# perdoch/hesaff

Measured on AMD Instinct MI355X. Metric: keypoints/sec (descriptors written), 4K grayscale batch, higher is better.
Workload: dtype f32

## Files before the change

hesaff_amd/csrc/kernels_patch.h:

```cpp
#pragma once
#include <type_traits>
#include "kernels_keypoint.h"

#define HS_PATCH_ARR 1684
#define HS_PATCH_PIX_IT 7
#define HS_NEED 82

struct PatchIO {
   DPlane image;
   float *patches;
   uint32_t h_base;
   float *trows;
   const uint32_t *row_prefix;
   uint32_t trows_cap;
   uint32_t *overflow;
};

__device__ __forceinline__ float hs_tap_inside(const HsPlaneBuf &im, float wx, float wy)
{
   const uint32_t off = ((uint32_t)(int)wy * im.pitch + (uint32_t)(int)wx) * 4u;
   wx = __builtin_amdgcn_fractf(wx);
   wy = __builtin_amdgcn_fractf(wy);
   const hs_v2u r0 = __builtin_amdgcn_raw_buffer_load_b64(im.rsrc, (int)off, 0, 0);
   const hs_v2u r1 = __builtin_amdgcn_raw_buffer_load_b64(im.rsrc, (int)off, (int)im.pitch_bytes, 0);
// ... 387 lines not shown
__device__ __forceinline__ void hs_resample_chunked(const float *__restrict__ T, int P, float scale, hs_row_taps taps, int r,
                                                    float *__restrict__ s_chunk, int chunk_rows, float *s_patch)
{
   const int tid = threadIdx.x;
   const float c0 = (float)(P >> 1);
   auto y0_of = [&](int jj) {
      const float wy = c0 + (float)(jj - (HS_PATCH >> 1)) * scale;
      return min(max((int)floorf(wy), 0), P - 2);
   };
   for (int jj0 = 0; jj0 < HS_PATCH;) {
      const int ylo = y0_of(jj0) - r;
      int jj1 = jj0;
      while (jj1 + 1 < HS_PATCH && y0_of(jj1 + 1) + r + 2 - ylo <= chunk_rows) jj1++;
      const int nrows = y0_of(jj1) + r + 2 - ylo;
      {
         const v2f *src = reinterpret_cast<const v2f *>(T + ylo * HS_NEED);
         v2f *dst = reinterpret_cast<v2f *>(s_chunk);
         const int n2 = nrows * (HS_NEED / 2);
#pragma unroll 4
         for (int i = tid; i < n2; i += 256) dst[i] = src[i];
      }
      __syncthreads();
      for (int idx = jj0 * HS_PATCH + tid; idx < (jj1 + 1) * HS_PATCH; idx += 256) {
         const int jj = hs_div_small(idx, 1.0f / (float)HS_PATCH), ii = idx - jj * HS_PATCH;
         const int j = jj - (HS_PATCH >> 1), i = ii - (HS_PATCH >> 1);
         const float rx = c0 + (float)j * 0.0f, ry = c0 + (float)j * scale;
         float wx = rx + (float)i * scale, wy = ry + (float)i * 0.0f;
         const float fx = floorf(wx), fy = floorf(wy);
         wx -= fx; wy -= fy;
         const int y0 = min(max((int)fy, 0), P - 2);
         const float *tc = s_chunk + (y0 - ylo) * HS_NEED + 2 * ii;
         auto ld = [&](int dy) { return *reinterpret_cast<const v2f *>(tc + dy * HS_NEED); };
         const v2f q0 = ld(0), q1 = ld(1);
         const float kc = taps[r];
         v2f da = kc * q0, db = kc * q1;
         v2f pj = q1, mj = q0;
#pragma unroll 4
         for (int jt = 1; jt <= r; jt++) {
            const v2f pn = ld(jt + 1), mn = ld(-jt);
            const float kj = taps[r + jt];
            const v2f sa = pj + mn, sb = pn + mj;
            da += kj * sa;
            db += kj * sb;
            pj = pn;
            mj = mn;
         }
         s_patch[idx] = (1.0f - wy) * ((1.0f - wx) * da.x + wx * da.y) + (wy) * ((1.0f - wx) * db.x + wx * db.y);
      }
      __syncthreads();
      jj0 = jj1 + 1;
   }
}

template <int NR, int NB>
__device__ __forceinline__ void hs_gather_slots(const HsPlaneBuf &img, const v2f *rc, const v2f *__restrict__ ctab, float a11, float a21, int half,
                                                int xb, int P, int r, float *__restrict__ srow, int sstride)
{
   const int lane = threadIdx.x & 63, pm = P - 1;
   float v[NR][NB];
#pragma unroll
   for (int it = 0; it < NB; it++) {
      const int xx = min(xb + lane + 64 * it, pm);
      const v2f c = ctab ? ctab[xx] : hs_col_coord(a11, a21, xx - half);
#pragma unroll
      for (int i = 0; i < NR; i++) {
         const v2f w = rc[i] + c;
         v[i][it] = hs_tap_inside(img, w.x, w.y);
      }
   }
#pragma unroll
   for (int it = 0; it < NB; it++)
#pragma unroll
      for (int i = 0; i < NR; i++) HS_KEEP(v[i][it]);
#pragma unroll
   for (int it = 0; it < NB; it++) {
      const int xx = xb + lane + 64 * it;
      if (xx < P) {
#pragma unroll
         for (int i = 0; i < NR; i++) srow[i * sstride + r + xx] = v[i][it];
      }
   }
}

template <int NR, int NIT>
__device__ __forceinline__ void hs_gather_rows(const HsPlaneBuf &img, const v2f *rc, const v2f *__restrict__ ctab, float a11, float a21, int half,
                                               int P, int r, float *__restrict__ srow, int sstride)
{
   static_assert(NIT == 1 || NIT == 2 || NIT == 4 || NIT == 8, "power of two");
   int xb = 0;
   for (; ((P - xb + 63) >> 6) >= NIT; xb += 64 * NIT)
      hs_gather_slots<NR, NIT>(img, rc, ctab, a11, a21, half, xb, P, r, srow, sstride);
   const int rem = (P - xb + 63) >> 6;
   if (NIT > 4 && (rem & 4)) { hs_gather_slots<NR, 4>(img, rc, ctab, a11, a21, half, xb, P, r, srow, sstride); xb += 256; }
   if (NIT > 2 && (rem & 2)) { hs_gather_slots<NR, 2>(img, rc, ctab, a11, a21, half, xb, P, r, srow, sstride); xb += 128; }
   if (NIT > 1 && (rem & 1)) { hs_gather_slots<NR, 1>(img, rc, ctab, a11, a21, half, xb, P, r, srow, sstride); }
}

template <int NIT>
__device__ __forceinline__ void hs_row_stream(const HsPlaneBuf &img, float x, float y, float a11, float a12, float a21, float a22, int P, int yy,
                                              float scale, const v2f *__restrict__ ctab, hs_row_taps taps, int K,
                                              float *__restrict__ srow, float *__restrict__ out82, int pad_r = 0)
{
   const int lane = threadIdx.x & 63, half = P >> 1, pm = P - 1, r = K >> 1;
   const v2f rc = hs_row_coord(x, y, a12, a22, yy - half);
   hs_gather_rows<1, NIT>(img, &rc, ctab, a11, a21, half, P, r, srow, 0);
   HS_WAVE_LDS_SYNC();
   {
      const float first = srow[r], last = srow[r + pm];
      for (int i = lane; i < r; i += 64) { srow[i] = first; srow[r + P + i] = last; }
   }
   HS_WAVE_LDS_SYNC();
   if (lane < HS_PATCH) {
      const float c0 = (float)half;
      const float w = c0 + (float)(lane - 20) * scale;
      const int x0 = min(max((int)floorf(w), 0), pm - 1);
      const float *s = srow + x0;
      auto G = [&](int jt) { v2f g; g.x = s[jt]; g.y = s[jt + 1]; return g; };
      v2f t = taps[0] * G(0);
#pragma unroll 8
      for (int jt = 1; jt < K; jt++) t += taps[jt] * G(jt);
      v2f *o = reinterpret_cast<v2f *>(out82) + lane;
      *o = t;
      if (pad_r > 0 && (yy == 0 || yy == pm)) {
         const int step = (yy == 0) ? -(HS_NEED / 2) : (HS_NEED / 2);
         for (int jr = 1; jr <= pad_r; jr++) o[jr * step] = t;
      }
   }
   HS_WAVE_LDS_SYNC();
}

template <int NIT>
__device__ __forceinline__ void hs_row_stream2(const HsPlaneBuf &img, float x, float y, float a12, float a22, int P, int yyA, int yyB,
                                               float scale, const v2f *__restrict__ ctab, hs_row_taps taps, int K,
                                               float *__restrict__ srowA, float *__restrict__ srowB, float *__restrict__ outA, float *__restrict__ outB, int pad_r,
                                               float a11 = 0.0f, float a21 = 0.0f)
{
   const int lane = threadIdx.x & 63, half = P >> 1, pm = P - 1, r = K >> 1;
   const v2f rc[2] = {hs_row_coord(x, y, a12, a22, yyA - half), hs_row_coord(x, y, a12, a22, yyB - half)};
   hs_gather_rows<2, NIT>(img, rc, ctab, a11, a21, half, P, r, srowA, (int)(srowB - srowA));
   HS_WAVE_LDS_SYNC();
   {
      const float fA = srowA[r], lA = srowA[r + pm], fB = srowB[r], lB = srowB[r + pm];
      for (int i = lane; i < r; i += 64) { srowA[i] = fA; srowA[r + P + i] = lA; srowB[i] = fB; srowB[r + P + i] = lB; }
   }
   HS_WAVE_LDS_SYNC();
   if (lane < HS_PATCH) {
      const float c0 = (float)half;
      const float w = c0 + (float)(lane - 20) * scale;
      const int x0 = min(max((int)floorf(w), 0), pm - 1);
      const float *sA = srowA + x0, *sB = srowB + x0;
      auto GA = [&](int jt) { v2f g; g.x = sA[jt]; g.y = sA[jt + 1]; return g; };
      auto GB = [&](int jt) { v2f g; g.x = sB[jt]; g.y = sB[jt + 1]; return g; };
      v2f tA = taps[0] * GA(0), tB = taps[0] * GB(0);
#pragma unroll 4
      for (int jt = 1; jt < K; jt++) {
         const float k = taps[jt];
         tA += k * GA(jt);
         tB += k * GB(jt);
      }
      v2f *oA = reinterpret_cast<v2f *>(outA) + lane, *oB = reinterpret_cast<v2f *>(outB) + lane;
      *oA = tA;
      *oB = tB;
      if (pad_r > 0 && yyA == 0)
         for (int jr = 1; jr <= pad_r; jr++) oA[-jr * (HS_NEED / 2)] = tA;
      if (pad_r > 0 && yyB == pm)
         for (int jr = 1; jr <= pad_r; jr++) oB[jr * (HS_NEED / 2)] = tB;
   }
   HS_WAVE_LDS_SYNC();
}

template <int NIT>
__device__ __forceinline__ void hs_row_stream3(const HsPlaneBuf &img, float x, float y, float a12, float a22, int P, int yy0, int yy1, int yy2,
                                               float scale, const v2f *__restrict__ ctab, hs_row_taps taps, int K,
                                               float *__restrict__ srow, int sstride, float *__restrict__ out0, float *__restrict__ out1,
                                               float *__restrict__ out2, int pad_r, float a11 = 0.0f, float a21 = 0.0f)
{
   const int lane = threadIdx.x & 63, half = P >> 1, pm = P - 1, r = K >> 1;
   const v2f rc[3] = {hs_row_coord(x, y, a12, a22, yy0 - half), hs_row_coord(x, y, a12, a22, yy1 - half),
                      hs_row_coord(x, y, a12, a22, yy2 - half)};
   float *srow1 = srow + sstride, *srow2 = srow + 2 * sstride;
   hs_gather_rows<3, NIT>(img, rc, ctab, a11, a21, half, P, r, srow, sstride);
   HS_WAVE_LDS_SYNC();
   {
      const float f0 = srow[r], l0 = srow[r + pm], f1 = srow1[r], l1 = srow1[r + pm], f2 = srow2[r], l2 = srow2[r + pm];
      for (int i = lane; i < r; i += 64) {
         srow[i] = f0; srow[r + P + i] = l0;
         srow1[i] = f1; srow1[r + P + i] = l1;
         srow2[i] = f2; srow2[r + P + i] = l2;
      }
   }
   HS_WAVE_LDS_SYNC();
   {
      const int tA = lane, tB = min(64 + lane, 3 * HS_PATCH - 1);
      const int rowA = tA >= HS_PATCH ? 1 : 0, rowB = tB >= 2 * HS_PATCH ? 2 : 1;
      const int colA = tA - HS_PATCH * rowA, colB = tB - HS_PATCH * rowB;
      const float c0 = (float)half;
      const float wA = c0 + (float)(colA - 20) * scale, wB = c0 + (float)(colB - 20) * scale;
      const int xA = min(max((int)floorf(wA), 0), pm - 1), xB = min(max((int)floorf(wB), 0), pm - 1);
      const float *sA = srow + rowA * sstride + xA, *sB = srow + rowB * sstride + xB;
      v2f tA2, tB2;
      float a0 = sA[0], a1 = sA[1], b0 = sB[0], b1 = sB[1];
      const float k0 = taps[0];
      float tA0 = k0 * a0, tA1 = k0 * a1, tB0 = k0 * b0, tB1 = k0 * b1;
#pragma unroll 4
      for (int jt = 1; jt < K; jt++) {
         const float k = taps[jt];
         a0 = a1; b0 = b1;
         a1 = sA[jt + 1]; b1 = sB[jt + 1];
         tA0 += k * a0; tA1 += k * a1;
         tB0 += k * b0; tB1 += k * b1;
      }
      tA2.x = tA0; tA2.y = tA1; tB2.x = tB0; tB2.y = tB1;
      const int yA = rowA ? yy1 : yy0, yB = rowB == 2 ? yy2 : yy1;
      v2f *oA = reinterpret_cast<v2f *>(rowA ? out1 : out0) + colA;
      v2f *oB = reinterpret_cast<v2f *>(rowB == 2 ? out2 : out1) + colB;
      *oA = tA2;
      if (64 + lane < 3 * HS_PATCH) *oB = tB2;
      if (pad_r > 0) {
         if (yA == 0) for (int jr = 1; jr <= pad_r; jr++) oA[-jr * (HS_NEED / 2)] = tA2;
         if (yA == pm) for (int jr = 1; jr <= pad_r; jr++) oA[jr * (HS_NEED / 2)] = tA2;
         if (64 + lane < 3 * HS_PATCH) {
            if (yB == 0) for (int jr = 1; jr <= pad_r; jr++) oB[-jr * (HS_NEED / 2)] = tB2;
            if (yB == pm) for (int jr = 1; jr <= pad_r; jr++) oB[jr * (HS_NEED / 2)] = tB2;
         }
      }
   }
   HS_WAVE_LDS_SYNC();
}

#define HS_MID_PMAX 128
#define HS_MID_SROW 160
#define HS_BIG_SROW 640
#define HS_BIG_TAPS 128
#define HS_MID_RPAD 14
#define HS_BIG_RPAD 57
#define HS_CHUNK_MIN_ROWS 4
#define HS_MID_NIT3_BIG 2
#define HS_MID_NIT3_SMALL 1
#define HS_MID_BLOCKS (256 * 7)
#define HS_BIG_BLOCKS (256 * 8)

template <int PMAX> struct MidGeom {
   static constexpr bool BIG = PMAX > HS_MID_PMAX;
   static constexpr int SROW = BIG ? HS_BIG_SROW : HS_MID_SROW;
   static constexpr int NTAP = BIG ? HS_BIG_TAPS : 32;
   static constexpr int RPAD = BIG ? HS_BIG_RPAD : HS_MID_RPAD;
   static constexpr int CHUNK_MIN = BIG ? 0 : 64;
   static constexpr int SROWS = 12 * SROW > CHUNK_MIN * HS_NEED ? 12 * SROW : CHUNK_MIN * HS_NEED;
   static constexpr int CHUNK_ROWS = SROWS / HS_NEED;
   static constexpr int FLOATS = HS_PATCH_ARR + NTAP + 2 * (PMAX + 2) + SROWS;
};

template <int PMAX>
__global__ __launch_bounds__(256) void k_patch_mid(HessList hl, PatchWork pw, PatchIO io, KpTables tb)
{
   typedef MidGeom<PMAX> GM;
   constexpr int BIN = GM::BIG ? 3 : 2;
   constexpr int NIT = GM::BIG ? 4 : 2;
   constexpr int NIT3 = GM::BIG ? HS_MID_NIT3_BIG : HS_MID_NIT3_SMALL;
   extern __shared__ __attribute__((aligned(16))) float smem[];
   float *s_patch = smem;
   v2f *s_C = reinterpret_cast<v2f *>(s_patch + HS_PATCH_ARR + GM::NTAP);
   float *s_srow = reinterpret_cast<float *>(s_C + (PMAX + 2));
   float *Tp = io.trows + (size_t)blockIdx.x * ((size_t)(PMAX + 2 * GM::RPAD) * HS_NEED);

   const int tid = threadIdx.x, wave = tid >> 6;
   const uint32_t cnt = min(pw.bin_count[BIN], pw.cap);
   const int imPitch = io.image.pitch;

   __shared__ uint32_t s_item;
   for (;;) {
      if (tid == 0) s_item = atomicAdd(pw.bin_work + BIN, 1u);
      __syncthreads();
      const uint32_t wi = (uint32_t)__builtin_amdgcn_readfirstlane((int)s_item);
      if (wi >= cnt) break;
      const uint32_t h = pw.bin_items[(size_t)BIN * pw.cap + wi];
      const int b = hl.meta[h] >> 8;
      const HsPlaneBuf ib = hs_plane_buf(io.image.img(b), io.image.rows, imPitch);
      const float x = hl.x[h], y = hl.y[h];
      const float a11 = pw.A[4 * h], a12 = pw.A[4 * h + 1], a21 = pw.A[4 * h + 2], a22 = pw.A[4 * h + 3];
      const int P0 = pw.P0[h], P = P0 + 2, half = P >> 1;
      const float scale = (float)P0 / (float)HS_PATCH;
      const int K = tb.patch_tap_k[(P0 - 1) >> 1];
      const float *taps_g = tb.patch_taps + tb.patch_tap_off[(P0 - 1) >> 1];
      const hs_row_taps ktap = HS_ROW_TAPS(taps_g);
      for (int m = tid; m < P; m += 256) s_C[m] = hs_col_coord(a11, a21, m - half);
      __syncthreads();
      float *srowA = s_srow + wave * 3 * GM::SROW, *srowB = srowA + GM::SROW;
#pragma unroll 1
      for (int yy = wave; yy < P; yy += 12) {
         const int rr = K >> 1;
         if (yy + 8 < P)
            hs_row_stream3<NIT3>(ib, x, y, a12, a22, P, yy, yy + 4, yy + 8, scale, s_C, ktap, K, srowA, GM::SROW,
                                 Tp + (size_t)(yy + rr) * HS_NEED, Tp + (size_t)(yy + 4 + rr) * HS_NEED, Tp + (size_t)(yy + 8 + rr) * HS_NEED, rr);
         else if (yy + 4 < P)
            hs_row_stream2<NIT>(ib, x, y, a12, a22, P, yy, yy + 4, scale, s_C, ktap, K, srowA, srowB,
                                Tp + (size_t)(yy + (K >> 1)) * HS_NEED, Tp + (size_t)(yy + 4 + (K >> 1)) * HS_NEED, K >> 1);
         else
            hs_row_stream<NIT>(ib, x, y, a11, a12, a21, a22, P, yy, scale, s_C, ktap, K, srowA,
                               Tp + (size_t)(yy + (K >> 1)) * HS_NEED, K >> 1);
      }
      __syncthreads();
      if ((float)(K + 1) + (float)(HS_CHUNK_MIN_ROWS - 1) * scale <= (float)GM::CHUNK_ROWS)
         hs_resample_chunked(Tp + (K >> 1) * HS_NEED, P, scale, ktap, K >> 1, s_srow, GM::CHUNK_ROWS, s_patch);
      else
         hs_resample_reduced_batched<true>(Tp + (K >> 1) * HS_NEED, P, scale, ktap, K >> 1, s_patch);
      __syncthreads();
      for (int i = tid; i < HS_PATCH_PIX; i += 256) {
         float *po = io.patches + (size_t)(h - io.h_base) * HS_PATCH_PIX + i;
         hs_store_nt(po, s_patch[i]);
      }
      __syncthreads();
   }
}

#define HS_LARGE_CHUNK 18
#define HS_LARGE_NIT3 2

__global__ __launch_bounds__(256) void k_patch_large_rows(HessList hl, PatchWork pw, PatchIO io, KpTables tb, int srow_stride, int tap_stride, int nrow,
                                                          int p_lo, int p_hi)
{
   extern __shared__ __attribute__((aligned(16))) float smem[];
   const int wave = __builtin_amdgcn_readfirstlane((int)(threadIdx.x >> 6));
   float *srow = smem + (size_t)wave * (nrow * srow_stride + tap_stride);
   const uint32_t *pre = io.row_prefix;
   const uint32_t n_items = min(pw.bin_count[HS_NBINS - 1], pw.cap);
   if (n_items == 0) return;
   const uint32_t row_hi = pre[n_items];
   if (row_hi > io.trows_cap) {
      if (threadIdx.x == 0 && blockIdx.x == 0) *io.overflow = 1u;
      return;
   }
   const int imPitch = io.image.pitch;
   const uint32_t ntasks = (row_hi + HS_LARGE_CHUNK - 1) / HS_LARGE_CHUNK;
   const uint32_t nw = blockDim.x >> 6;
   for (uint32_t task = blockIdx.x * nw + wave; task < ntasks; task += gridDim.x * nw) {
      uint32_t row = task * HS_LARGE_CHUNK;
      const uint32_t row_end = min(row + HS_LARGE_CHUNK, row_hi);
      uint32_t lo = 0, hi = n_items;
      while (hi - lo > 1) {
         const uint32_t mid = (lo + hi) >> 1;
         if (pre[mid] <= row) lo = mid; else hi = mid;
      }
      uint32_t it = lo;
      while (row < row_end) {
         const uint32_t it_rows_end = min(pre[it + 1], row_end);
         const uint32_t h = pw.bin_items[(size_t)(HS_NBINS - 1) * pw.cap + it];
         const int P0 = pw.P0[h], P = P0 + 2;
         if (P <= p_lo || P > p_hi) { row = it_rows_end; it++; continue; }
         const int b = hl.meta[h] >> 8;
         const float scale = (float)P0 / (float)HS_PATCH;
         const int K = tb.patch_tap_k[(P0 - 1) >> 1];
         const float *taps = tb.patch_taps + tb.patch_tap_off[(P0 - 1) >> 1];
         const HsPlaneBuf ib = hs_plane_buf(io.image.img(b), io.image.rows, imPitch);
         const float kx = hl.x[h], ky = hl.y[h];
         const float a11 = pw.A[4 * h], a12 = pw.A[4 * h + 1], a21 = pw.A[4 * h + 2], a22 = pw.A[4 * h + 3];
         const uint32_t first = pre[it];
         const hs_row_taps ktap = HS_ROW_TAPS(taps);
         float *const out0 = io.trows + (size_t)row * HS_NEED;
// ... 105 lines not shown
```

hesaff_amd/csrc/pipeline.hip:

```cpp
#include <hip/hip_runtime.h>
#include <algorithm>
#include <atomic>
#include <chrono>
#include <cmath>
#include <cstdio>
#include <cstdlib>
#include <cstring>
#include <string>
#include <vector>
#include <condition_variable>
#include <deque>
#include <future>
#include <map>
#include <memory>
#include <mutex>
#include <thread>

#include "../../include/hesaff_amd.h"
#include "host_tables.h"
#include "kernels_keypoint.h"
#include "kernels_patch.h"
#include "kernels_sift.h"
#include "kernels_pyramid.h"
#include "kernels_export.h"
// ... 275 lines not shown
         if (bytes == 0 || bytes > kLargest) return nullptr;
         std::vector<std::pair<void *, size_t>> evicted;
         bool room = false;
         {
            std::lock_guard<std::mutex> lk(mu);
            for (size_t k = 0; k < parked.size(); k++)
               if (parked[k].second == bytes) { void *q = parked[k].first; parked[k] = parked.back(); parked.pop_back(); return q; }
            while (bytes_total + bytes > max_bytes && !parked.empty()) {
               evicted.push_back(parked.back());
               bytes_total -= parked.back().second;
               parked.pop_back();
            }
            room = bytes_total + bytes <= max_bytes;
            if (room) bytes_total += bytes;
         }
         for (auto &b : evicted) (void)hipHostFree(b.first);
         if (!room) return nullptr;
         void *q = nullptr;
         if (hipSetDevice(device) != hipSuccess || hipHostMalloc(&q, bytes, hipHostMallocDefault) != hipSuccess) {
            (void)hipGetLastError();
            std::lock_guard<std::mutex> lk(mu);
            bytes_total -= bytes;
            return nullptr;
         }
         return q;
      }
      void give(void *q, size_t bytes)
      {
         std::lock_guard<std::mutex> lk(mu);
         parked.emplace_back(q, bytes);
      }
      void trim(size_t keep)
      {
         std::vector<std::pair<void *, size_t>> out;
         {
            std::lock_guard<std::mutex> lk(mu);
            size_t held = 0;
            for (auto &b : parked) held += b.second;
            while (held > keep && !parked.empty()) {
               out.push_back(parked.back());
               held -= parked.back().second; bytes_total -= parked.back().second;
               parked.pop_back();
            }
         }
         for (auto &b : out) (void)hipHostFree(b.first);
      }
      ~PinReadCache() { trim(0); }
   } pin_read;
   std::vector<PinBuf> pin_out;
   hesaff_engine::BlockRing ring;
   hipStream_t h2d_stream = nullptr, d2h_stream = nullptr;
   float export_ms = 0.0f; int32_t export_rows = 0;
   PinBuf h_small_end, h_small_mid, h_small_exp;
   DevBuf t_mask_idx, t_sgrad_nb, t_sgrad_om, t_vo_rows, t_vo_src, b_rowprefix, b_trows, b_trows2, b_trows3;
   DevBuf b_jplane;
   DevBuf b_ex_len, b_ex_sums, b_ex_off, b_ex_imgoff, b_ex_starts;
   size_t rows_lds_set = 0;
   int n_cu = 256;
   uint32_t g_small0 = 256 * 6, g_small1 = 256 * 4, g_mid = HS_MID_BLOCKS, g_big = HS_BIG_BLOCKS, g_lfin = 256 * 4, g_shist = 256 * 32;
   uint32_t sgrad_grid = 256 * 32;
   uint32_t trows_rows = 4u << 20;

   hesaff_timings tm;
   int profiling = 0;
   int out_format = HESAFF_OUT_TEXT;
   int resume = 0;
   int pool_priority = -1;
   int stage_threads = 4;
   hipStream_t side_streams[HS_NSIDE] = {nullptr, nullptr, nullptr, nullptr};
   hipStream_t sift_stream = nullptr;
   hipStream_t aff_stream = nullptr;
   DevEvent ev_detect_done, ev_batch_done;
   std::vector<DevEvent> ev_aff;
   DevEvent ev_extract_done[HS_NSLOT], ev_sift_done[HS_NSLOT];
   DevBuf b_patches2[HS_NSLOT];
   DevBuf b_siftvec2, b_meanvar2, b_siftvo2;
   DevEvent ev_fork, ev_join[HS_NSIDE];
   bool fast_pyramid = false;
   bool no_overlap = false;
   bool debug = false;

   std::vector<DevEvent> ev_pool;
   size_t ev_used = 0;
};

namespace {

struct EvPair { hipEvent_t a, b; int kind; double bytes; };

hipEvent_t get_event(hesaff_ctx *c)
{
   if (c->ev_used == c->ev_pool.size()) c->ev_pool.emplace_back(hipEventDefault);
   return c->ev_pool[c->ev_used++];
}

template <class T> void upload(DevBuf &b, const std::vector<T> &v)
{
   b.ensure(std::max<size_t>(v.size() * sizeof(T), 16));
   HIP_TRY(hipMemcpy(b.p, v.data(), v.size() * sizeof(T), hipMemcpyHostToDevice));
}

void build_tables(hesaff_ctx *c)
{
   std::vector<float> smm(HS_SMM_PIX), sm(HS_PATCH_PIX), w0(HS_PATCH), w1(HS_PATCH);
   std::vector<int32_t> b0(HS_PATCH), b1(HS_PATCH);
   hesaff::gauss_mask(HS_SMM, smm.data());
   hesaff::circ_gauss_mask(HS_PATCH, sm.data());
// ... 209 lines not shown
         }
   }
   const int ppitch0 = round_up(PW, 64);
   const size_t pplane0 = (size_t)B * PH * ppitch0;
   if (c->up) {
      c->geo.b_up.ensure(pplane0 * 4);
      c->upimg = make_plane(c->geo.b_up.as<float>(), PH, PW, ppitch0);
   }
   c->geo.b_L3.ensure(pplane0 * 4);
   c->geo.b_R.ensure(pplane0 * 4 * 5);
   {
      const void *before = c->geo.b_map.p;
      const size_t before_bytes = c->geo.b_map.bytes;
      c->geo.b_map.ensure(std::max<size_t>((size_t)B * PH * PW * 4, 16));
      if (c->geo.b_map.p != before || c->geo.b_map.bytes != before_bytes) c->map_clean = false;
      int kb = 1;
      while (kb < 32 && (3ull * (unsigned long long)PH * PW) > (1ull << kb)) kb++;
      if (kb != c->map_kbits) { c->map_kbits = kb; c->map_clean = false; }
   }
   const long long total_words = (long long)B * words;
   c->geo.b_bitmask.ensure(std::max<size_t>((size_t)total_words * 8, 16));
   c->geo.b_prefix.ensure(std::max<size_t>((size_t)(total_words + 1) * 4, 16));
   double mpx = (double)B * PH * PW / 1.0e6;
   double capd = mpx * (double)c->par.max_kpts_per_mpx;
   if (capd < 4096) capd = 4096;
   if (capd > 2.0e9) throw HsError(HESAFF_ERR_ARG, "batch too large for 32-bit keypoint indices");
   c->cap = ((uint32_t)capd + 63u) & ~63u;
   const size_t cap = c->cap;
   const long long scan_items = std::max<long long>(total_words, (long long)cap);
   c->geo.b_blocksums.ensure((size_t)((scan_items + SCAN_BLOCK - 1) / SCAN_BLOCK + 1) * 4);
   c->b_counters.ensure(64 * 4);
   {
      const unsigned long long waves0 = (unsigned long long)((PW + EXM_STRIP - 1) / EXM_STRIP) * (unsigned long long)(PH / 32 + 1) * (unsigned long long)B;
      const unsigned long long cc = (unsigned long long)cap + (unsigned long long)cap / 8 + HS_CAND_BLOCK * waves0;
      if (cc > 0xfffffff0ull) throw HsError(HESAFF_ERR_ARG, "batch too large for 32-bit candidate indices");
      c->cand_cap = (uint32_t)cc;
      c->geo.b_cand.ensure((size_t)cc * sizeof(CandRec));
   }
   c->geo.b_rec_f.ensure(cap * 4 * 4);
   c->geo.b_rec_i.ensure(cap * 4 * 4);
   c->geo.b_rec_w.ensure(cap * 8);
   c->geo.b_hess_f.ensure(cap * 4 * 4);
   c->geo.b_hess_i.ensure(cap * 2 * 4);
   c->geo.b_aff.ensure(cap * 6 * 4);
   c->geo.b_pw.ensure(cap * 6 * 4);
   c->geo.b_bins.ensure(cap * HS_NBINS * 4);
   c->geo.b_rank.ensure((cap + 1) * 4);
   c->geo.b_desc.ensure(cap * 128);
   c->geo.b_out.ensure(cap * sizeof(KeyRec));
   c->geo.b_starts.ensure(((size_t)(B + 1) * 3 + 2) * 4);
   const int max_p0 = (int)std::floor(std::sqrt((double)W * (double)H)) + 3;
   ensure_patch_taps(c, max_p0);
   refresh_tables_struct(c);
   c->b_trows2.ensure((size_t)HS_MID_BLOCKS * (HS_MID_PMAX + 2 * HS_MID_RPAD) * HS_NEED * 4);
   c->b_trows3.ensure((size_t)HS_BIG_BLOCKS * (HS_BIN3_PMAX + 2 * HS_BIG_RPAD) * HS_NEED * 4);
   {
      const LargeGeom lg = large_geom(c->max_p0 + 2);
      if (lg.lds / 4 > HS_LDS_PER_CU) throw HsError(HESAFF_ERR_ARG, "image too large for the large-window row kernel (sqrt(width x height) above about 27900)");
      const size_t want = std::min<size_t>(lg.lds + (size_t)8 * lg.srow_stride * 4, HS_LDS_PER_CU);
      if (want > c->rows_lds_set) {
         set_dyn_lds(k_patch_large_rows, want);
         c->rows_lds_set = want;
      }
   }
   c->B = B; c->H = H; c->W = W;
}

template <class LOAD> void exclusive_scan(hesaff_ctx *c, LOAD load, long long n, uint32_t *out, uint32_t *total)
{
   if (n <= 0) { HIP_TRY(hipMemsetAsync(total, 0, 4, c->stream)); return; }
   const int nb = (int)((n + SCAN_BLOCK - 1) / SCAN_BLOCK);
   uint32_t *bs = c->geo.b_blocksums.as<uint32_t>();
   hipLaunchKernelGGL(k_scan_reduce<LOAD>, dim3(nb), dim3(256), 0, c->stream, load, n, bs);
   hipLaunchKernelGGL(k_scan_sums, dim3(1), dim3(256), 0, c->stream, bs, nb, total);
   hipLaunchKernelGGL(k_scan_down<LOAD>, dim3(nb), dim3(256), 0, c->stream, load, n, bs, out);
}

struct StageTimer {
   hesaff_ctx *c;
   std::vector<EvPair> pairs;
   std::vector<hipStream_t> streams;
   explicit StageTimer(hesaff_ctx *ctx) : c(ctx) {}
   int begin(int kind, double bytes = 0, hipStream_t st = nullptr)
   {
      if (!c->profiling) return -1;
      if (kind >= 100 && c->profiling < 2) return -1;
      if (!st) st = c->stream;
      EvPair p; p.a = get_event(c); p.b = get_event(c); p.kind = kind; p.bytes = bytes;
      (void)hipEventRecord(p.a, st);
      pairs.push_back(p);
      streams.push_back(st);
      return (int)pairs.size() - 1;
   }
   void end(int id) { if (id >= 0) (void)hipEventRecord(pairs[id].b, streams[id]); }
};

enum { T_PYR = 0, T_DET = 1, T_AFF = 2, T_PATCH = 3, T_SIFT = 4, T_TOTAL = 5, T_PACK = 6, T_BLURHESS = 100, T_EXTREMA = 101 };

template <int K, bool WL, bool WR, bool WH, bool WR0 = false, int SRC = SRC_PLANE>
void launch_march(hesaff_ctx *c, const DPlane &in, const DPlane &outL, const DPlane &outR, const DPlane &outHalf, const float *taps,
                  float norm2, int B, const DPlane &outR0 = DPlane(), float norm2_in = 0.0f, const GraySrc &gs = GraySrc(), const DPlane &outGray = DPlane())
{
   const int strips = (in.cols + BM_STRIP - 1) / BM_STRIP;
   const long long blocks_per_band = (long long)((strips + 3) / 4) * B;
   int best_nb = 16 * (int)std::max<long long>(1, std::min<long long>(4, 64 / std::max<long long>(1, blocks_per_band)));
   best_nb = std::max(1, std::min(best_nb, std::max(1, in.rows / 8)));
   const int band = (in.rows + best_nb - 1) / best_nb;
// ... 58 lines not shown
   uint32_t *cnt = c->b_counters.as<uint32_t>();
   const size_t cap = c->cap;
   s.counters = cnt;
   s.cl.count = cnt + 0; s.cl.items = c->geo.b_cand.as<CandRec>(); s.cl.cap = c->cand_cap; s.cl.overflow = cnt + 2;
   s.rl.count = cnt + 1; s.rl.cap = c->cap;
   float *rf = c->geo.b_rec_f.as<float>();
   s.rl.x = rf; s.rl.y = rf + cap; s.rl.s = rf + 2 * cap; s.rl.response = rf + 3 * cap;
   uint32_t *ri = c->geo.b_rec_i.as<uint32_t>();
   s.rl.meta = (int32_t *)ri; s.rl.cell = ri + cap; s.rl.key = ri + 2 * cap; s.rl.bit = ri + 3 * cap;
   s.rl.word = c->geo.b_rec_w.as<long long>();
   float *hf = c->geo.b_hess_f.as<float>();
   s.hl.x = hf; s.hl.y = hf + cap; s.hl.s = hf + 2 * cap; s.hl.response = hf + 3 * cap;
   int32_t *hi = c->geo.b_hess_i.as<int32_t>();
   s.hl.meta = hi; s.hl.r0c0 = hi + cap; s.hl.cap = c->cap;
   int32_t *ai = c->geo.b_aff.as<int32_t>();
   s.ao.converged = ai; s.ao.iters = ai + cap; s.ao.U = (float *)(ai + 2 * cap);
   int32_t *pi = c->geo.b_pw.as<int32_t>();
   s.pw.P0 = pi; s.pw.alive = pi + cap; s.pw.A = (float *)(pi + 2 * cap);
   s.pw.bin_count = cnt + 8; s.pw.bin_work = cnt + 24; s.pw.bin_items = c->geo.b_bins.as<uint32_t>(); s.pw.cap = c->cap;
   return s;
}

void run_patch_stage(hesaff_ctx *c, const Lists &s, const DPlane &image, float *patches_out, uint32_t h_base, uint32_t large_rows_bound,
                     const PlaneTab *pt = nullptr)
{
   hipStream_t st = c->stream;
   PatchIO io;
   memset(&io, 0, sizeof io);
   io.image = image;
   io.patches = patches_out;
   io.h_base = h_base;
   if (c->fast_pyramid && pt) {
      hipStream_t s0 = st;
      const bool forked = c->side_streams[0] && !c->no_overlap;
      if (forked) {
         HIP_TRY(hipEventRecord(c->ev_fork, st));
         HIP_TRY(hipStreamWaitEvent(c->side_streams[0], c->ev_fork, 0));
         s0 = c->side_streams[0];
      }
      hipLaunchKernelGGL(k_patch_extract_small<0>, dim3(c->g_small0), dim3(256), small_extract_lds_bytes(0), s0, s.hl, s.pw, io, c->tables);
      if (forked) HIP_TRY(hipEventRecord(c->ev_join[0], s0));
      hipLaunchKernelGGL(k_patch_pyramid, dim3((uint32_t)c->n_cu * 32u), dim3(256), 0, st, s.hl, s.pw, io, *pt, (int)c->oct.size(), c->consts.pd0, 1);
      if (forked) HIP_TRY(hipStreamWaitEvent(st, c->ev_join[0], 0));
      return;
   }
   hipStream_t s0 = st, s1 = st, s2 = st, s3 = st;
   const bool forked = c->side_streams[0] && !c->no_overlap;
   if (forked) {
      HIP_TRY(hipEventRecord(c->ev_fork, st));
      for (int i = 0; i < HS_NSIDE; i++) HIP_TRY(hipStreamWaitEvent(c->side_streams[i], c->ev_fork, 0));
      s0 = c->side_streams[0]; s1 = c->side_streams[1]; s2 = c->side_streams[2]; s3 = c->side_streams[3];
   }
   {
      PatchIO io2 = io;
      io2.trows = c->b_trows2.as<float>();
      PatchIO io3 = io;
      io3.trows = c->b_trows3.as<float>();
      hipLaunchKernelGGL(k_patch_extract_small<0>, dim3(c->g_small0), dim3(256), small_extract_lds_bytes(0), s0, s.hl, s.pw, io, c->tables);
      hipLaunchKernelGGL(k_patch_extract_small<1>, dim3(c->g_small1), dim3(256), small_extract_lds_bytes(1), s1, s.hl, s.pw, io, c->tables);
      hipLaunchKernelGGL(k_patch_mid<HS_MID_PMAX>, dim3(c->g_mid), dim3(256), mid_lds_bytes(), s2, s.hl, s.pw, io2, c->tables);
      hipLaunchKernelGGL(k_patch_mid<HS_BIN3_PMAX>, dim3(c->g_big), dim3(256), big_lds_bytes(), s3, s.hl, s.pw, io3, c->tables);
   }
   if (large_rows_bound > 0) {
      const uint32_t rows_cap = std::max(large_rows_bound, c->trows_rows);
      c->b_trows.ensure((size_t)rows_cap * HS_NEED * 4);
      c->b_rowprefix.ensure(((size_t)c->cap + 1) * 4);
      const int pmax = std::min(c->max_p0 + 2, std::max(HS_BIN3_PMAX + 1, (c->batch_max_p > 0 ? c->batch_max_p : c->max_p0 + 2)));
      io.trows = c->b_trows.as<float>();
      io.row_prefix = c->b_rowprefix.as<uint32_t>();
      io.trows_cap = rows_cap;
      io.overflow = s.counters + 6;
      hipLaunchKernelGGL(k_large_prefix, dim3(1), dim3(256), 0, st, s.pw, c->b_rowprefix.as<uint32_t>());
      auto launch_rows = [&](int p_lo, int p_hi) {
         const LargeGeom lg = large_geom(std::min(c->max_p0 + 2, (p_hi + 255) / 256 * 256));
         const size_t wave1 = lg.lds / 4;
         const size_t wave3 = wave1 + (size_t)2 * lg.srow_stride * 4;
         const int nrow = wave3 * 6 <= HS_LDS_PER_CU ? 3 : 1;
         const size_t per_wave = nrow == 3 ? wave3 : wave1;
         uint32_t nw = 4;
         while (nw > 1 && per_wave * nw > HS_LDS_PER_CU) nw >>= 1;
         if (nw == 4 && (HS_LDS_PER_CU / (per_wave * 2)) * 2 > (HS_LDS_PER_CU / (per_wave * 4)) * 4) nw = 2;
         if (nrow == 3) nw = std::min<uint32_t>(nw, HS_LARGE_NW);
         const uint32_t gblocks = std::min<uint32_t>((large_rows_bound + nw * HS_LARGE_CHUNK - 1) / (nw * HS_LARGE_CHUNK), 256 * 16 * (4 / nw));
         hipLaunchKernelGGL(k_patch_large_rows, dim3(gblocks), dim3(64 * nw), per_wave * nw, st, s.hl, s.pw, io, c->tables, lg.srow_stride, lg.tap_stride, nrow,
                            p_lo, std::min(p_hi, 0x7ffffff0));
      };
      if (pmax > HS_LARGE_SPLIT) { launch_rows(0, HS_LARGE_SPLIT); launch_rows(HS_LARGE_SPLIT, pmax); }
      else launch_rows(0, pmax);
      hipLaunchKernelGGL(k_patch_large_finish, dim3(c->g_lfin), dim3(256), 0, st, s.pw, io, c->tables);
   }
   if (forked) {
      for (int i = 0; i < HS_NSIDE; i++) HIP_TRY(hipEventRecord(c->ev_join[i], c->side_streams[i]));
      for (int i = 0; i < HS_NSIDE; i++) HIP_TRY(hipStreamWaitEvent(st, c->ev_join[i], 0));
   }
}

void run_detection(hesaff_ctx *c, const SrcImages &src, int B, const Lists &s, StageTimer &tm, bool keep_all_planes, float *planes_out,
                   bool detect = true)
{
   const hesaff::OctaveSchedule &sc = c->sched;
   hipStream_t st = c->stream;
   uint32_t *cnt = s.counters;
   const float *ptaps = c->t_pyr_taps.as<float>();
   if (detect) {
      HIP_TRY(hipMemsetAsync(cnt, 0, 64 * 4, st));
      HIP_TRY(hipMemsetAsync(c->geo.b_bitmask.p, 0, std::max<size_t>((size_t)B * c->words_per_image * 8, 8), st));
      if (!c->map_clean) { HIP_TRY(hipMemsetAsync(c->geo.b_map.p, 0xFF, c->geo.b_map.bytes, st)); c->map_epoch = c->map_kbits < 32 ? (0xffffffffu >> c->map_kbits) : 0u; c->map_clean = true; }
   }

   int t = tm.begin(T_PYR);
   DPlane none = make_plane(nullptr, 0, 0, 0);
   const bool fused_gray = !c->oct.empty() && c->pyr_K[0] == 11 && !c->up;
   if (fused_gray) {
// ... 441 lines not shown
```

Before: 38.69 million.

## Keep mid-bin transposed rows in an LDS ring and resample incrementally

For the mid-size patch kernel, the row-filtered intermediate rows are now kept in a sliding LDS window instead of a per-block global scratch buffer. Output patch rows are resampled from that window as soon as their source rows are ready, and the live rows are compacted to the front when the window fills. This removes the global write/readback round trip and the mid trows allocation. In exchange it adds extra block-wide barriers and copy passes, and it uses more LDS per block, which the code asserts still allows five blocks per CU.

Result: no change. 38.66 million (-0.1%).

```diff
diff --git a/hesaff_amd/csrc/kernels_patch.h b/hesaff_amd/csrc/kernels_patch.h
--- a/hesaff_amd/csrc/kernels_patch.h
+++ b/hesaff_amd/csrc/kernels_patch.h
@@ -463,6 +463,41 @@
    }
 }
 
+template <bool TAIL>
+__device__ __forceinline__ void hs_resample_rows_lds(const float *__restrict__ s_T, int base, int jj0, int jj1, int P, float scale, hs_row_taps taps,
+                                                     int r, float *s_patch)
+{
+   const float c0 = (float)(P >> 1);
+   for (int idx = jj0 * HS_PATCH + (int)threadIdx.x; idx < (jj1 + 1) * HS_PATCH; idx += 256) {
+      const int jj = hs_div_small(idx, 1.0f / (float)HS_PATCH), ii = idx - jj * HS_PATCH;
+      const int j = jj - (HS_PATCH >> 1), i = ii - (HS_PATCH >> 1);
+      const float rx = c0 + (float)j * 0.0f, ry = c0 + (float)j * scale;
+      float wx = rx + (float)i * scale, wy = ry + (float)i * 0.0f;
+      const float fx = floorf(wx), fy = floorf(wy);
+      wx -= fx; wy -= fy;
+      const int y0 = min(max((int)fy, 0), P - 2);
+      const float *tc = s_T + (y0 + r - base) * HS_NEED + 2 * ii;
+      const int dmax = P - 1 - y0;
+      auto ld = [&](int dy) { return *reinterpret_cast<const v2f *>(tc + dy * HS_NEED); };
+      auto ldp = [&](int dy) { return ld(TAIL ? min(dy, dmax) : dy); };
+      const v2f q0 = ld(0), q1 = ld(1);
+      const float kc = taps[r];
+      v2f da = kc * q0, db = kc * q1;
+      v2f pj = q1, mj = q0;
+#pragma unroll 4
+      for (int jt = 1; jt <= r; jt++) {
+         const v2f pn = ldp(jt + 1), mn = ld(-jt);
+         const float kj = taps[r + jt];
+         const v2f sa = pj + mn, sb = pn + mj;
+         da += kj * sa;
+         db += kj * sb;
+         pj = pn;
+         mj = mn;
+      }
+      s_patch[idx] = (1.0f - wy) * ((1.0f - wx) * da.x + wx * da.y) + (wy) * ((1.0f - wx) * db.x + wx * db.y);
+   }
+}
+
 template <int NR, int NB>
 __device__ __forceinline__ void hs_gather_slots(const HsPlaneBuf &img, const v2f *rc, const v2f *__restrict__ ctab, float a11, float a21, int half,
                                                 int xb, int P, int r, float *__restrict__ srow, int sstride)
@@ -510,7 +545,7 @@
 template <int NIT>
 __device__ __forceinline__ void hs_row_stream(const HsPlaneBuf &img, float x, float y, float a11, float a12, float a21, float a22, int P, int yy,
                                               float scale, const v2f *__restrict__ ctab, hs_row_taps taps, int K,
-                                              float *__restrict__ srow, float *__restrict__ out82, int pad_r = 0)
+                                              float *__restrict__ srow, float *__restrict__ out82, int pad_r = 0, bool pad_below = true)
 {
    const int lane = threadIdx.x & 63, half = P >> 1, pm = P - 1, r = K >> 1;
    const v2f rc = hs_row_coord(x, y, a12, a22, yy - half);
@@ -532,7 +567,7 @@
       for (int jt = 1; jt < K; jt++) t += taps[jt] * G(jt);
       v2f *o = reinterpret_cast<v2f *>(out82) + lane;
       *o = t;
-      if (pad_r > 0 && (yy == 0 || yy == pm)) {
+      if (pad_r > 0 && (yy == 0 || (pad_below && yy == pm))) {
          const int step = (yy == 0) ? -(HS_NEED / 2) : (HS_NEED / 2);
          for (int jr = 1; jr <= pad_r; jr++) o[jr * step] = t;
       }
@@ -544,7 +579,7 @@
 __device__ __forceinline__ void hs_row_stream2(const HsPlaneBuf &img, float x, float y, float a12, float a22, int P, int yyA, int yyB,
                                                float scale, const v2f *__restrict__ ctab, hs_row_taps taps, int K,
                                                float *__restrict__ srowA, float *__restrict__ srowB, float *__restrict__ outA, float *__restrict__ outB, int pad_r,
-                                               float a11 = 0.0f, float a21 = 0.0f)
+                                               float a11 = 0.0f, float a21 = 0.0f, bool pad_below = true)
 {
    const int lane = threadIdx.x & 63, half = P >> 1, pm = P - 1, r = K >> 1;
    const v2f rc[2] = {hs_row_coord(x, y, a12, a22, yyA - half), hs_row_coord(x, y, a12, a22, yyB - half)};
@@ -574,7 +609,7 @@
       *oB = tB;
       if (pad_r > 0 && yyA == 0)
          for (int jr = 1; jr <= pad_r; jr++) oA[-jr * (HS_NEED / 2)] = tA;
-      if (pad_r > 0 && yyB == pm)
+      if (pad_r > 0 && pad_below && yyB == pm)
          for (int jr = 1; jr <= pad_r; jr++) oB[jr * (HS_NEED / 2)] = tB;
    }
    HS_WAVE_LDS_SYNC();
@@ -584,7 +619,8 @@
 __device__ __forceinline__ void hs_row_stream3(const HsPlaneBuf &img, float x, float y, float a12, float a22, int P, int yy0, int yy1, int yy2,
                                                float scale, const v2f *__restrict__ ctab, hs_row_taps taps, int K,
                                                float *__restrict__ srow, int sstride, float *__restrict__ out0, float *__restrict__ out1,
-                                               float *__restrict__ out2, int pad_r, float a11 = 0.0f, float a21 = 0.0f)
+                                               float *__restrict__ out2, int pad_r, float a11 = 0.0f, float a21 = 0.0f,
+                                               bool pad_below = true)
 {
    const int lane = threadIdx.x & 63, half = P >> 1, pm = P - 1, r = K >> 1;
    const v2f rc[3] = {hs_row_coord(x, y, a12, a22, yy0 - half), hs_row_coord(x, y, a12, a22, yy1 - half),
@@ -629,10 +665,10 @@
       if (64 + lane < 3 * HS_PATCH) *oB = tB2;
       if (pad_r > 0) {
          if (yA == 0) for (int jr = 1; jr <= pad_r; jr++) oA[-jr * (HS_NEED / 2)] = tA2;
-         if (yA == pm) for (int jr = 1; jr <= pad_r; jr++) oA[jr * (HS_NEED / 2)] = tA2;
+         if (pad_below && yA == pm) for (int jr = 1; jr <= pad_r; jr++) oA[jr * (HS_NEED / 2)] = tA2;
          if (64 + lane < 3 * HS_PATCH) {
             if (yB == 0) for (int jr = 1; jr <= pad_r; jr++) oB[-jr * (HS_NEED / 2)] = tB2;
-            if (yB == pm) for (int jr = 1; jr <= pad_r; jr++) oB[jr * (HS_NEED / 2)] = tB2;
+            if (pad_below && yB == pm) for (int jr = 1; jr <= pad_r; jr++) oB[jr * (HS_NEED / 2)] = tB2;
          }
       }
    }
@@ -648,18 +684,22 @@
 #define HS_CHUNK_MIN_ROWS 4
 #define HS_MID_NIT3_BIG 2
 #define HS_MID_NIT3_SMALL 1
+#define HS_MID_TROWS 52
 #define HS_MID_BLOCKS (256 * 7)
 #define HS_BIG_BLOCKS (256 * 8)
 
 template <int PMAX> struct MidGeom {
    static constexpr bool BIG = PMAX > HS_MID_PMAX;
    static constexpr int SROW = BIG ? HS_BIG_SROW : HS_MID_SROW;
-   static constexpr int NTAP = BIG ? HS_BIG_TAPS : 32;
    static constexpr int RPAD = BIG ? HS_BIG_RPAD : HS_MID_RPAD;
-   static constexpr int CHUNK_MIN = BIG ? 0 : 64;
-   static constexpr int SROWS = 12 * SROW > CHUNK_MIN * HS_NEED ? 12 * SROW : CHUNK_MIN * HS_NEED;
+   static constexpr int SROWS = 12 * SROW;
    static constexpr int CHUNK_ROWS = SROWS / HS_NEED;
-   static constexpr int FLOATS = HS_PATCH_ARR + NTAP + 2 * (PMAX + 2) + SROWS;
+   static constexpr int NTAP = BIG ? HS_BIG_TAPS : 0;
+   static constexpr int TROWS = BIG ? 0 : HS_MID_TROWS;
+   static constexpr int COPY_IT = ((2 * RPAD + 1) * (HS_NEED / 2) + 255) / 256;
+   static constexpr int FLOATS = HS_PATCH_ARR + NTAP + 2 * (PMAX + 2) + SROWS + TROWS * HS_NEED;
+   static_assert(BIG || TROWS >= 2 * RPAD + 1 + 12, "a round's rows beside the live ones");
+   static_assert(BIG || FLOATS * 4 + 256 <= 160 * 1024 / 5, "five blocks per CU");
 };
 
 template <int PMAX>
@@ -673,8 +713,8 @@
    float *s_patch = smem;
    v2f *s_C = reinterpret_cast<v2f *>(s_patch + HS_PATCH_ARR + GM::NTAP);
    float *s_srow = reinterpret_cast<float *>(s_C + (PMAX + 2));
-   float *Tp = io.trows + (size_t)blockIdx.x * ((size_t)(PMAX + 2 * GM::RPAD) * HS_NEED);
-
+   float *Tp = nullptr;
+   if constexpr (GM::BIG) Tp = io.trows + (size_t)blockIdx.x * ((size_t)(PMAX + 2 * GM::RPAD) * HS_NEED);
    const int tid = threadIdx.x, wave = tid >> 6;
    const uint32_t cnt = min(pw.bin_count[BIN], pw.cap);
    const int imPitch = io.image.pitch;
@@ -698,24 +738,71 @@
       for (int m = tid; m < P; m += 256) s_C[m] = hs_col_coord(a11, a21, m - half);
       __syncthreads();
       float *srowA = s_srow + wave * 3 * GM::SROW, *srowB = srowA + GM::SROW;
+      if constexpr (!GM::BIG) {
+         float *s_T = s_srow + GM::SROWS;
+         const int r = K >> 1;
+         const float c0 = (float)half;
+         auto y0_of = [&](int jj) {
+            const float wy = c0 + (float)(jj - (HS_PATCH >> 1)) * scale;
+            return min(max((int)floorf(wy), 0), P - 2);
+         };
+         int base = 0;
+         int jjn = 0;
 #pragma unroll 1
-      for (int yy = wave; yy < P; yy += 12) {
-         const int rr = K >> 1;
-         if (yy + 8 < P)
-            hs_row_stream3<NIT3>(ib, x, y, a12, a22, P, yy, yy + 4, yy + 8, scale, s_C, ktap, K, srowA, GM::SROW,
-                                 Tp + (size_t)(yy + rr) * HS_NEED, Tp + (size_t)(yy + 4 + rr) * HS_NEED, Tp + (size_t)(yy + 8 + rr) * HS_NEED, rr);
-         else if (yy + 4 < P)
-            hs_row_stream2<NIT>(ib, x, y, a12, a22, P, yy, yy + 4, scale, s_C, ktap, K, srowA, srowB,
-                                Tp + (size_t)(yy + (K >> 1)) * HS_NEED, Tp + (size_t)(yy + 4 + (K >> 1)) * HS_NEED, K >> 1);
+         for (int yb = 0; yb < P; yb += 12) {
+            if (yb + r + 12 - base > GM::TROWS) {
+               const int nbase = y0_of(jjn);
+               const int n2 = (yb + r - nbase) * (HS_NEED / 2);
+               const v2f *src = reinterpret_cast<const v2f *>(s_T + (nbase - base) * HS_NEED);
+               v2f *dst = reinterpret_cast<v2f *>(s_T);
+               v2f keep[GM::COPY_IT];
+#pragma unroll
+               for (int k = 0; k < GM::COPY_IT; k++)
+                  if (tid + 256 * k < n2) keep[k] = src[tid + 256 * k];
+               __syncthreads();
+#pragma unroll
+               for (int k = 0; k < GM::COPY_IT; k++)
+                  if (tid + 256 * k < n2) dst[tid + 256 * k] = keep[k];
+               base = nbase;
+            }
+            const int yy = yb + wave;
+            float *o = s_T + (yy + r - base) * HS_NEED;
+            if (yy + 8 < P)
+               hs_row_stream3<NIT3>(ib, x, y, a12, a22, P, yy, yy + 4, yy + 8, scale, s_C, ktap, K, srowA, GM::SROW,
+                                    o, o + 4 * HS_NEED, o + 8 * HS_NEED, r, 0.0f, 0.0f, false);
+            else if (yy + 4 < P)
+               hs_row_stream2<NIT>(ib, x, y, a12, a22, P, yy, yy + 4, scale, s_C, ktap, K, srowA, srowB, o, o + 4 * HS_NEED, r, 0.0f, 0.0f, false);
+            else if (yy < P)
+               hs_row_stream<NIT>(ib, x, y, a11, a12, a21, a22, P, yy, scale, s_C, ktap, K, srowA, o, r, false);
+            __syncthreads();
+            if (yb + 12 < P) {
+               int jj1 = jjn - 1;
+               while (jj1 + 1 < HS_PATCH && y0_of(jj1 + 1) + r + 1 <= yb + 11) jj1++;
+               if (jj1 >= jjn) hs_resample_rows_lds<false>(s_T, base, jjn, jj1, P, scale, ktap, r, s_patch);
+               jjn = jj1 + 1;
+            } else
+               hs_resample_rows_lds<true>(s_T, base, jjn, HS_PATCH - 1, P, scale, ktap, r, s_patch);
+         }
+      } else {
+#pragma unroll 1
+         for (int yy = wave; yy < P; yy += 12) {
+            const int rr = K >> 1;
+            if (yy + 8 < P)
+               hs_row_stream3<NIT3>(ib, x, y, a12, a22, P, yy, yy + 4, yy + 8, scale, s_C, ktap, K, srowA, GM::SROW,
+                                    Tp + (size_t)(yy + rr) * HS_NEED, Tp + (size_t)(yy + 4 + rr) * HS_NEED, Tp + (size_t)(yy + 8 + rr) * HS_NEED, rr);
+            else if (yy + 4 < P)
+               hs_row_stream2<NIT>(ib, x, y, a12, a22, P, yy, yy + 4, scale, s_C, ktap, K, srowA, srowB,
+                                   Tp + (size_t)(yy + (K >> 1)) * HS_NEED, Tp + (size_t)(yy + 4 + (K >> 1)) * HS_NEED, K >> 1);
+            else
+               hs_row_stream<NIT>(ib, x, y, a11, a12, a21, a22, P, yy, scale, s_C, ktap, K, srowA,
+                                  Tp + (size_t)(yy + (K >> 1)) * HS_NEED, K >> 1);
+         }
+         __syncthreads();
+         if ((float)(K + 1) + (float)(HS_CHUNK_MIN_ROWS - 1) * scale <= (float)GM::CHUNK_ROWS)
+            hs_resample_chunked(Tp + (K >> 1) * HS_NEED, P, scale, ktap, K >> 1, s_srow, GM::CHUNK_ROWS, s_patch);
          else
-            hs_row_stream<NIT>(ib, x, y, a11, a12, a21, a22, P, yy, scale, s_C, ktap, K, srowA,
-                               Tp + (size_t)(yy + (K >> 1)) * HS_NEED, K >> 1);
-      }
-      __syncthreads();
-      if ((float)(K + 1) + (float)(HS_CHUNK_MIN_ROWS - 1) * scale <= (float)GM::CHUNK_ROWS)
-         hs_resample_chunked(Tp + (K >> 1) * HS_NEED, P, scale, ktap, K >> 1, s_srow, GM::CHUNK_ROWS, s_patch);
-      else
-         hs_resample_reduced_batched<true>(Tp + (K >> 1) * HS_NEED, P, scale, ktap, K >> 1, s_patch);
+            hs_resample_reduced_batched<true>(Tp + (K >> 1) * HS_NEED, P, scale, ktap, K >> 1, s_patch);
+      }
       __syncthreads();
       for (int i = tid; i < HS_PATCH_PIX; i += 256) {
          float *po = io.patches + (size_t)(h - io.h_base) * HS_PATCH_PIX + i;
diff --git a/hesaff_amd/csrc/pipeline.hip b/hesaff_amd/csrc/pipeline.hip
--- a/hesaff_amd/csrc/pipeline.hip
+++ b/hesaff_amd/csrc/pipeline.hip
@@ -351,7 +351,7 @@
    hipStream_t h2d_stream = nullptr, d2h_stream = nullptr;
    float export_ms = 0.0f; int32_t export_rows = 0;
    PinBuf h_small_end, h_small_mid, h_small_exp;
-   DevBuf t_mask_idx, t_sgrad_nb, t_sgrad_om, t_vo_rows, t_vo_src, b_rowprefix, b_trows, b_trows2, b_trows3;
+   DevBuf t_mask_idx, t_sgrad_nb, t_sgrad_om, t_vo_rows, t_vo_src, b_rowprefix, b_trows, b_trows3;
    DevBuf b_jplane;
    DevBuf b_ex_len, b_ex_sums, b_ex_off, b_ex_imgoff, b_ex_starts;
    size_t rows_lds_set = 0;
@@ -667,7 +667,6 @@
    const int max_p0 = (int)std::floor(std::sqrt((double)W * (double)H)) + 3;
    ensure_patch_taps(c, max_p0);
    refresh_tables_struct(c);
-   c->b_trows2.ensure((size_t)HS_MID_BLOCKS * (HS_MID_PMAX + 2 * HS_MID_RPAD) * HS_NEED * 4);
    c->b_trows3.ensure((size_t)HS_BIG_BLOCKS * (HS_BIN3_PMAX + 2 * HS_BIG_RPAD) * HS_NEED * 4);
    {
       const LargeGeom lg = large_geom(c->max_p0 + 2);
@@ -832,13 +831,11 @@
       s0 = c->side_streams[0]; s1 = c->side_streams[1]; s2 = c->side_streams[2]; s3 = c->side_streams[3];
    }
    {
-      PatchIO io2 = io;
-      io2.trows = c->b_trows2.as<float>();
       PatchIO io3 = io;
       io3.trows = c->b_trows3.as<float>();
       hipLaunchKernelGGL(k_patch_extract_small<0>, dim3(c->g_small0), dim3(256), small_extract_lds_bytes(0), s0, s.hl, s.pw, io, c->tables);
       hipLaunchKernelGGL(k_patch_extract_small<1>, dim3(c->g_small1), dim3(256), small_extract_lds_bytes(1), s1, s.hl, s.pw, io, c->tables);
-      hipLaunchKernelGGL(k_patch_mid<HS_MID_PMAX>, dim3(c->g_mid), dim3(256), mid_lds_bytes(), s2, s.hl, s.pw, io2, c->tables);
+      hipLaunchKernelGGL(k_patch_mid<HS_MID_PMAX>, dim3(c->g_mid), dim3(256), mid_lds_bytes(), s2, s.hl, s.pw, io, c->tables);
       hipLaunchKernelGGL(k_patch_mid<HS_BIN3_PMAX>, dim3(c->g_big), dim3(256), big_lds_bytes(), s3, s.hl, s.pw, io3, c->tables);
    }
    if (large_rows_bound > 0) {
```
